# JosephCatrambone/aruco3

Measured on AMD Instinct MI355X. Metric: frames/sec at 1920x1080 ARUCO dict, higher is better.
Workload: dtype u8

## Files before the change

aruco3_amd/csrc/a3_api.hip:

```cpp
#include <algorithm>
#include <atomic>
#include <cmath>
#include <chrono>
#include <cstddef>
#include <cstdio>
#include <cstring>
#include <mutex>
#include <string>
#include <vector>

#include "a3_common.h"
#include "a3_internal.h"
#include "a3_launch.h"
#include "a3_readback.h"
#include "a3_solve_check.h"

using namespace a3;

namespace {

thread_local std::string g_create_error;

constexpr uint32_t kMaxCandDefault = 1024, kMaxCandLimit = A3_MAX_CANDIDATES_PER_FRAME;
static_assert(kMaxCandLimit == 65536, "a3_marker.candidate_index is a uint16_t");
// ... 116 lines not shown
    bool grey_valid = false;
    bool contours_valid = false;
    uint32_t tap_contours = 0; uint64_t tap_points = 0;
    bool markers_valid = false;
    uint32_t last_n = 0, last_max_per_frame = 0;
    int profiling = 0;
    int profile_every = 1;
    uint32_t batch_seq = 0;
    hipEvent_t ev[6] = {nullptr, nullptr, nullptr, nullptr, nullptr, nullptr};
    double prof_ms[A3_STAGE_COUNT] = {0, 0, 0};
    uint64_t prof_n[A3_STAGE_COUNT] = {0, 0, 0};
    a3_stats stats{};

    uint32_t W = 0, H = 0, frames = 0;

    DevBuf dict, in, grey, bin, frame_darts, frame_darts_dev, frame_base, pix_base, tile_darts;
    DevBuf d_xy, d_succ, fin, t_cur, t_next;
    DevBuf leader_list, leader_keep, entry_list, es_a, es_b;
    DevBuf contours, cyc_start_off, points;
    DevBuf cands, pre_xy, fin_xy, fin_count, work, outs, proj, patches, cand_big;
    DevBuf zero_blk;
    a3_marker* markers_ptr = nullptr;
    unsigned long long* frame_darts_ptr = nullptr;
    unsigned int* scratch_u32 = nullptr; DeviceCounters* counters = nullptr; uint32_t* per_frame = nullptr; uint32_t* frame_cursor = nullptr; uint32_t* cand_count = nullptr;
    uint32_t last_marker_total = 0;
    DevBuf tmp_a, tmp_b, tmp_c, tmp_d;
    DevBuf hsum;
    DevBuf wtab;
    DevBuf pose_buf;
    bool poses_valid = false;
    a3_refine_config refine{};
    a3_refine_config refine_prm_cfg{};
// ... 83 lines not shown
    if (bytes <= ctx->pinned_cap) return A3_OK;
    if (ctx->pinned) (void)hipHostFree(ctx->pinned);
    ctx->pinned = nullptr; ctx->pinned_cap = 0;
    A3_HIP(hipHostMalloc(&ctx->pinned, bytes, hipHostMallocDefault));
    ctx->pinned_cap = bytes;
    return A3_OK;
}

uint32_t mark_size_of(uint8_t num_bits) {
    return (uint32_t)((uint8_t)std::ceil(std::sqrt((float)num_bits)) + 2);
}

int ensure_dart_pool(a3_ctx* ctx, uint64_t darts) {
    A3_HIP(ctx->d_xy.ensure(darts * 8));
    A3_HIP(ctx->d_succ.ensure(darts * 4));
    A3_HIP(ctx->fin.ensure(darts * fin_state_bytes()));
    A3_HIP(ctx->t_cur.ensure(darts * 8));
    A3_HIP(ctx->t_next.ensure(darts * 8));
    A3_HIP(ctx->leader_list.ensure(leader_list_bytes((uint32_t)darts)));
    A3_HIP(ctx->leader_keep.ensure(leader_list_bytes((uint32_t)darts)));
    const size_t eslots = entry_slots((uint32_t)darts);
    A3_HIP(ctx->entry_list.ensure(eslots * 4));
    A3_HIP(ctx->es_a.ensure(eslots * entry_state_bytes()));
    A3_HIP(ctx->es_b.ensure(eslots * entry_state_bytes()));
    return A3_OK;
}

struct DeviceStreams { hipStream_t decode = nullptr, copy = nullptr; };
std::mutex g_streams_mu;
DeviceStreams g_dev_streams[64];
// ... 246 lines not shown
        if (b.want_pose && b.undist) A3_HIP(ctx->charuco_und.ensure(std::max<size_t>(recs, 1) * 8));
    }
    if (int rc = ensure_pinned(ctx, pinned_bytes(b.rb))) return rc;
    if (b.taps && ctx->pinned_counts_cap < (size_t)b.n * 8) {
        if (ctx->pinned_counts) (void)hipHostFree(ctx->pinned_counts);
        ctx->pinned_counts = nullptr; ctx->pinned_counts_cap = 0;
        A3_HIP(hipHostMalloc(&ctx->pinned_counts, (size_t)b.n * 8, hipHostMallocDefault));
        ctx->pinned_counts_cap = (size_t)b.n * 8;
    }
    return A3_OK;
}
int ensure_chain_buffers(a3_ctx* ctx, hipStream_t st, Batch& b, uint64_t cap_d) {
    const uint32_t n = b.n;
    const ZeroLayout z = zero_layout(1, n, n, b.marker_cap);
    A3_HIP(ctx->tile_darts.ensure(tile_darts_bytes(b.W, b.H, n)));
    A3_HIP(ctx->zero_blk.ensure(z.total));
    if (ctx->frame_darts_dev.cap < (size_t)n * 8) {
        A3_HIP(ctx->frame_darts_dev.ensure((size_t)n * 8));
        A3_HIP(hipMemsetAsync(ctx->frame_darts_dev.p, 0, ctx->frame_darts_dev.cap, st));
    }
    A3_HIP(ctx->frame_base.ensure((size_t)(n + 1) * 4));
    if (int rc = ensure_dart_pool(ctx, pool_darts_of(ctx, cap_d, 1))) return rc;
    A3_HIP(ctx->pix_base.ensure((size_t)n * b.W * b.H * 4));
    A3_HIP(ctx->contours.ensure((size_t)ctx->max_contours * sizeof(ContourRec)));
    A3_HIP(ctx->cyc_start_off.ensure((size_t)ctx->max_contours * 4));
    A3_HIP(ctx->points.ensure(ctx->max_points * 4));
    return ensure_back_buffers(ctx, b, z.head_bytes);
}


int enqueue_front(a3_ctx* ctx, Batch& b, bool held) {
    hipStream_t st = ctx->stream;
    const uint32_t n = b.n, W = b.W, H = b.H;
    const size_t npx = (size_t)W * H;
    const uint32_t kMaxCand = ctx->max_cand;
    const bool big_window = threshold_writes_grey_plane(ctx->cfg.threshold_window);
    b.need_grey = b.taps || big_window;
    b.grey_src = big_window || (b.taps && !b.sample_frames);
// ... 24 lines not shown
    if (b.prof) A3_HIP(hipEventRecord(ctx->ev[0], st));
    A3_HIP(launch_grey_threshold(st, {.pixels = b.pixels, .fmt = b.fmt, .row_stride = b.row_stride, .frame_stride = b.frame_stride, .W = (int)W, .H = (int)H,
                                      .n = n, .radius = ctx->cfg.threshold_window, .grey = b.need_grey ? ctx->grey.as<uint8_t>() : nullptr,
                                      .bits = ctx->bin.as<uint64_t>(), .hsum_tmp = big_window ? ctx->hsum.as<uint16_t>() : nullptr}));
    if (b.prof) A3_HIP(hipEventRecord(ctx->ev[1], st));
    if (!held) return A3_OK;
    A3_HIP(hipEventRecord(ctx->ev_k1_done, st));
    const uint64_t cap_d = device_plan_capacity(ctx, n, W, H);
    if (cap_d == 0) return fail(ctx, A3_ERR_INTERNAL, "a chain was held back for a batch that needs a host-side plan");
    return ensure_chain_buffers(ctx, st, b, cap_d);
}

ContourChunk contour_chunk(const a3_ctx* ctx) {
    ContourChunk c;
    c.W = (int)ctx->W; c.H = (int)ctx->H; c.batch_frames = ctx->frames;
    c.bits = ctx->bin.as<uint64_t>(); c.tile_darts = ctx->tile_darts.as<uint32_t>(); c.pix_base = ctx->pix_base.as<uint32_t>();
    c.d_rec = ctx->d_xy.as<uint64_t>(); c.d_succ = ctx->d_succ.as<uint32_t>();
    c.entry_list = ctx->entry_list.as<uint32_t>(); c.es_a = ctx->es_a.p; c.es_b = ctx->es_b.p; c.fin = ctx->fin.p;
    c.leader_count = ctx->scratch_u32 + 16; c.entry_count = ctx->scratch_u32 + 32;
    c.leader_list = ctx->leader_list.as<uint32_t>(); c.leader_keep = ctx->leader_keep.as<uint32_t>();
    c.t_cur = ctx->t_cur.as<uint64_t>(); c.t_next = ctx->t_next.as<uint64_t>();
    c.contours = ctx->contours.as<ContourRec>(); c.cyc_start_off = ctx->cyc_start_off.as<uint32_t>(); c.points = ctx->points.as<uint32_t>();
    c.max_contours = ctx->max_contours; c.max_points = ctx->max_points;
    c.cands = ctx->cands.as<CandRec>(); c.cand_count = ctx->cand_count;
    c.err_flags = ctx->scratch_u32 + 4;
    return c;
}

int enqueue_chain(a3_ctx* ctx, Batch& b, bool defer_locked) {
    hipStream_t st = ctx->stream;
    const uint32_t n = b.n, W = b.W, H = b.H;
// ... 35 lines not shown
        ctx->counters = reinterpret_cast<DeviceCounters*>(z + head_off + 256);
        ctx->per_frame = reinterpret_cast<uint32_t*>(z + head_off + 256 + ctr_bytes);
        ctx->markers_ptr = reinterpret_cast<a3_marker*>(z + head_off + head_bytes);
        zero_p = z; zero_bytes = (head_off + head_bytes + 15) & ~(size_t)15;
        return launch ? launch_zero(st, zero_p, zero_bytes) : hipSuccess;
    };
    std::vector<Chunk> chunks;
    std::vector<uint64_t> fd;
    if (device_plan) {
        if (int rc = ensure_chain_buffers(ctx, st, b, cap_d)) return rc;
        chunks.push_back(Chunk{0, n, cap_d, (uint32_t)std::min<uint64_t>(cap_d, 0xFFFFFFFFu)});
        A3_HIP(layout_zero_block(1, n, false));
        ctx->frame_darts_ptr = ctx->frame_darts_dev.as<unsigned long long>();
    } else {
        A3_HIP(ctx->tile_darts.ensure(tile_darts_bytes(W, H, n)));
        ctx->frame_darts_ptr = ctx->frame_darts.as<unsigned long long>();
        A3_HIP(hipMemsetAsync(ctx->frame_darts.p, 0, (size_t)n * 8, st));
    }
    DartCountLaunch count{.bits = ctx->bin.as<uint64_t>(), .W = (int)W, .H = (int)H, .n_frames = n, .frame_darts = ctx->frame_darts_ptr,
                          .tile_darts = ctx->tile_darts.as<uint32_t>(), .plan_cap = cap_d};
    if (device_plan) { count.frame_base = ctx->frame_base.as<uint32_t>(); count.plan = ctx->scratch_u32 + 8; count.zero_p = zero_p; count.zero_bytes = zero_bytes; }
    A3_HIP(launch_dart_count(st, count));
    const uint32_t* n_live = device_plan ? ctx->scratch_u32 + 8 : nullptr;
    uint32_t max_chunk_frames = n;
    if (!device_plan) {
        if (int rc = ensure_pinned(ctx, std::max<size_t>((size_t)n * 8, 1 << 16))) return rc;
        A3_HIP(hipMemcpyAsync(ctx->pinned, ctx->frame_darts.p, (size_t)n * 8, hipMemcpyDeviceToHost, st));
        A3_HIP(wait_stream(st));
        fd.assign((uint64_t*)ctx->pinned, (uint64_t*)ctx->pinned + n);
        uint64_t biggest = 0;
        for (uint64_t v : fd) { biggest = std::max(biggest, v); ctx->stats.darts += v; }
        if (biggest > kHardMaxDarts) return fail(ctx, A3_ERR_LIMIT, "a frame needs more contour-graph nodes than 32-bit indices allow");
        if (biggest > ctx->max_darts) ctx->max_darts = biggest;
        Chunk c{0, 0, 0, 0};
        for (uint32_t f = 0; f < n; f++) {
            if (c.count && (c.darts + fd[f] > ctx->max_darts || c.count >= kMaxChunkFrames)) { chunks.push_back(c); c = Chunk{f, 0, 0, 0}; }
            c.count++; c.darts += fd[f]; c.max_frame_darts = (uint32_t)std::max<uint64_t>(c.max_frame_darts, fd[f]);
        }
        if (c.count) chunks.push_back(c);
        max_chunk_frames = 0; uint64_t max_chunk_darts = 0;
        for (auto& c : chunks) { max_chunk_frames = std::max(max_chunk_frames, c.count); max_chunk_darts = std::max(max_chunk_darts, c.darts); }
        if (int rc = ensure_dart_pool(ctx, pool_darts_of(ctx, max_chunk_darts, chunks.size()))) return rc;
        A3_HIP(ctx->pix_base.ensure((size_t)max_chunk_frames * npx * 4));
        A3_HIP(ctx->frame_base.ensure((size_t)(max_chunk_frames + 1) * 4 * chunks.size()));
        A3_HIP(layout_zero_block(chunks.size(), max_chunk_frames, true));
        A3_HIP(ctx->contours.ensure((size_t)ctx->max_contours * sizeof(ContourRec)));
        A3_HIP(ctx->cyc_start_off.ensure((size_t)ctx->max_contours * 4));
        A3_HIP(ctx->points.ensure(ctx->max_points * 4));
        std::vector<uint32_t> bases;
        for (auto& c : chunks) {
            uint32_t acc = 0;
            for (uint32_t i = 0; i < max_chunk_frames + 1; i++) {
                bases.push_back(acc);
                if (i < c.count) acc += (uint32_t)fd[c.first + i];
            }
        }
        if (int rc = ensure_pinned(ctx, (size_t)n * 8 + bases.size() * 4 + (1 << 16))) return rc;
        uint32_t* h_bases = reinterpret_cast<uint32_t*>((uint8_t*)ctx->pinned + (size_t)n * 8);
// ... 390 lines not shown
        for (size_t i = 0; i < g_deferred.size(); i++)
            if (g_deferred[i] == ctx) { g_deferred.erase(g_deferred.begin() + (long)i); break; }
        ctx->back_deferred = false;
        for (size_t i = 0; i < g_held.size(); i++)
            if (g_held[i] == ctx) { g_held.erase(g_held.begin() + (long)i); break; }
        ctx->rest_held = false;
    }
    if (ctx->stream && ctx->stream != ctx->own_stream) (void)hipStreamSynchronize(ctx->stream);
    {
        DeviceStreams ds;
        { std::lock_guard<std::mutex> lk(g_streams_mu); ds = g_dev_streams[ctx->device & 63]; }
        if (ds.decode) (void)hipStreamSynchronize(ds.decode);
        if (ds.copy) (void)hipStreamSynchronize(ds.copy);
    }
    if (ctx->own_stream) (void)hipStreamSynchronize(ctx->own_stream);
    DevBuf* bufs[] = {&ctx->dict, &ctx->in, &ctx->grey, &ctx->bin, &ctx->frame_darts, &ctx->frame_darts_dev, &ctx->frame_base, &ctx->pix_base,
                      &ctx->tile_darts, &ctx->d_xy, &ctx->d_succ, &ctx->fin, &ctx->t_cur, &ctx->t_next,
                      &ctx->leader_list, &ctx->leader_keep, &ctx->entry_list, &ctx->es_a, &ctx->es_b,
                      &ctx->contours, &ctx->cyc_start_off, &ctx->points, &ctx->zero_blk, &ctx->cands,
                      &ctx->pre_xy, &ctx->fin_xy, &ctx->fin_count, &ctx->work, &ctx->outs, &ctx->proj, &ctx->patches, &ctx->cand_big,
                      &ctx->tmp_a, &ctx->tmp_b, &ctx->tmp_c, &ctx->tmp_d, &ctx->hsum, &ctx->pose_buf, &ctx->wtab, &ctx->refined_buf,
                      &ctx->board_slot_of, &ctx->board_slot_rec, &ctx->board_buf, &ctx->undist_buf, &ctx->charuco_tab, &ctx->charuco_tmp,
                      &ctx->charuco_buf, &ctx->charuco_und, &ctx->charuco_pose_buf, &ctx->solve_in,
                      &ctx->solve_scratch, &ctx->solve_big, &ctx->solve_out, &ctx->rect_in, &ctx->rect_out};
    for (DevBuf* b : bufs) b->release();
    if (ctx->pinned) (void)hipHostFree(ctx->pinned);
    if (ctx->pinned_counts) (void)hipHostFree(ctx->pinned_counts);
    for (auto& ev : ctx->ev) if (ev) (void)hipEventDestroy(ev);
    if (ctx->ev_in) (void)hipEventDestroy(ctx->ev_in);
    if (ctx->ev_contours) (void)hipEventDestroy(ctx->ev_contours);
    if (ctx->ev_k1) (void)hipEventDestroy(ctx->ev_k1);
    if (ctx->ev_gate) (void)hipEventDestroy(ctx->ev_gate);
// ... 325 lines not shown
    for (int r = 0; r < reps; r++) {
        A3_HIP(hipMemsetAsync(cc.leader_count, 0, 4 * 32, st));
        A3_HIP(hipEventRecord(e0, st));
        if (kernel == 0) {
            A3_HIP(hipMemsetAsync(ctx->frame_darts.p, 0, (size_t)ctx->frames * 8, st));
            A3_HIP(launch_dart_count(st, {.bits = cc.bits, .W = cc.W, .H = cc.H, .n_frames = ctx->frames, .frame_darts = ctx->frame_darts.as<unsigned long long>(),
                                          .tile_darts = ctx->tile_darts.as<uint32_t>()}));
        } else if (kernel == 1) {
            cc.dbg = dbg ? dbg : 5;
            A3_HIP(launch_dart_build(st, cc));
        } else if (kernel == 2) {
            cc.dbg = dbg ? dbg : 11;
            A3_HIP(launch_rank_cycles(st, cc));
        } else if (kernel == 3 || kernel == 4) {
            if (kernel == 4) {
                const size_t sweep = std::min<size_t>(ctx->pix_base.cap & ~(size_t)15, (size_t)512 << 20);
                if (sweep) A3_HIP(launch_zero(st, ctx->pix_base.p, sweep));
                A3_HIP(hipEventRecord(e0, st));
            }
            DecodeStage dec = decode_stage(ctx);
            dec.src = ctx->dbg_src; dec.W = cc.W; dec.H = cc.H; dec.max_cand = ctx->max_cand; dec.few = ctx->frames <= 64u; dec.grid_blocks = 4096;
            dec.per_frame = nullptr;
            dec.projection = dbg >= 0; dec.variant = dbg < 0 ? -dbg : dbg;
            A3_HIP(launch_decode(st, dec));
        } else return fail(ctx, A3_ERR_INVALID, "kernel: 0 dart_count, 1 dart_assign, 2 local_contract, 3 decode, 4 decode on cold frames");
        A3_HIP(hipEventRecord(e1, st));
        A3_HIP(hipStreamSynchronize(ctx->stream));
        float ms = 0;
        A3_HIP(hipEventElapsedTime(&ms, e0, e1));
        total += ms;
    }
    *avg_ms = (float)(total / reps);
// ... 1016 lines not shown
```

aruco3_amd/csrc/a3_launch.h:

```cpp
#pragma once

#include "a3_common.h"

namespace a3 {

struct ThresholdLaunch {
    const uint8_t* pixels = nullptr; int fmt = 0; size_t row_stride = 0, frame_stride = 0; int W = 0, H = 0; uint32_t n = 0, radius = 0;
    uint8_t* grey = nullptr; uint64_t* bits = nullptr; uint16_t* hsum_tmp = nullptr;
};
hipError_t launch_grey_threshold(hipStream_t st, const ThresholdLaunch& t);
bool threshold_writes_grey_plane(uint32_t radius);
hipError_t launch_k1_r1(hipStream_t st, const ThresholdLaunch& t);
hipError_t launch_k1_r2(hipStream_t st, const ThresholdLaunch& t);
bool ring_kernel_applies(uint32_t radius);
hipError_t launch_ring_threshold(hipStream_t st, const ThresholdLaunch& t);

size_t tile_darts_bytes(uint32_t W, uint32_t H, uint32_t n_frames);
struct DartCountLaunch {
    const uint64_t* bits = nullptr; int W = 0, H = 0; uint32_t first_frame = 0, n_frames = 0; unsigned long long* frame_darts = nullptr;
    uint32_t* tile_darts = nullptr; uint64_t plan_cap = 0; uint32_t* frame_base = nullptr; uint32_t* plan = nullptr; void* zero_p = nullptr;
    size_t zero_bytes = 0;
};
hipError_t launch_dart_count(hipStream_t st, const DartCountLaunch& d);
hipError_t launch_zero(hipStream_t st, void* p, size_t bytes);

size_t entry_state_bytes();
size_t fin_state_bytes();
size_t entry_slots(uint32_t n_darts);
size_t leader_list_bytes(uint32_t n_darts);

struct ContourChunk {
    uint32_t first_frame = 0, n_frames = 0, n_darts = 0; const uint32_t* frame_base = nullptr; DeviceCounters* ctr = nullptr;
    int max_rounds = 0;
    uint32_t* frame_entries = nullptr;
    unsigned int* dead_count = nullptr;
    int W = 0, H = 0;
    uint32_t batch_frames = 0;
    const uint64_t* bits = nullptr; const uint32_t* tile_darts = nullptr;
    const uint32_t* n_live = nullptr;
    uint32_t* pix_base = nullptr; uint64_t* d_rec = nullptr; uint32_t* d_succ = nullptr; uint32_t* entry_list = nullptr;
    unsigned int* entry_count = nullptr, * leader_count = nullptr;
    void* es_a = nullptr, * es_b = nullptr;
    void* fin = nullptr;
    uint32_t* leader_list = nullptr, * leader_keep = nullptr; uint64_t* t_cur = nullptr, * t_next = nullptr;
    int resolve_iters = 0;
    int inline_resolve_W = 0;
    uint32_t min_edge_length = 0; double eps_factor = 0.0; ContourRec* contours = nullptr; uint32_t* cyc_start_off = nullptr;
    uint32_t* points = nullptr; uint32_t max_contours = 0; uint64_t max_points = 0;
    bool keep_all = false;
    CandRec* cands = nullptr;
    uint32_t* cand_count = nullptr; uint32_t max_cand = 0; unsigned int* err_flags = nullptr;
    int phase = 0, dbg = 0;
};
hipError_t launch_dart_build(hipStream_t st, const ContourChunk& c);
hipError_t launch_rank_cycles(hipStream_t st, const ContourChunk& c);
// ... 128 lines not shown
```

aruco3_amd/csrc/k_contours.hip:

```cpp
#include <algorithm>
#include <cmath>

#include "a3_common.h"
#include "a3_launch.h"


namespace a3 {

constexpr int kFinB = 8;
constexpr int kScatB = 1;

struct Nb8 { uint64_t c; uint64_t n[8]; };

__device__ __forceinline__ uint64_t ldw(const uint64_t* __restrict__ img, int wpr, int H, int j, int y) {
    return (y >= 0 && y < H && j >= 0 && j < wpr) ? img[(size_t)y * wpr + j] : 0ull;
}

__device__ __forceinline__ void pdart_words(const Nb8& nb, uint64_t p[8]) {
#pragma unroll
    for (int k = 0; k < 8; k++) {
        uint64_t m = nb.c & nb.n[k] & ~nb.n[(k + 7) & 7];
        if ((k & 1) == 0) m &= ~nb.n[(k + 6) & 7];
        p[k] = m;
    }
// ... 11 lines not shown
    A3_DPP_ADD(0x143, 0xC)
#undef A3_DPP_ADD
    if (lane == 63) s_wave[wave] = inc;
    __syncthreads();
    uint32_t base = 0, tot = 0;
#pragma unroll
    for (int w = 0; w < 4; w++) {
        const uint32_t t = s_wave[w];
        if (w < wave) base += t;
        tot += t;
    }
    *total = tot;
    return base + inc - v;
}

constexpr int kTileWords = 4, kTileRows = 64;
__host__ __device__ inline uint32_t dart_tiles_x(uint32_t W) { return (words_per_row(W) + kTileWords - 1) / kTileWords; }
__host__ __device__ inline uint32_t dart_tiles(uint32_t W, uint32_t H) { return dart_tiles_x(W) * ((H + kTileRows - 1) / kTileRows); }

__device__ __forceinline__ void tile_stage(const uint64_t* __restrict__ img, int W, int H, uint32_t tile, uint64_t (*s_t)[kTileWords + 2]) {
    const int wpr = (int)words_per_row((uint32_t)W);
    const int tx = tile % dart_tiles_x((uint32_t)W), ty = tile / dart_tiles_x((uint32_t)W);
    const int j0 = tx * kTileWords - 1, y0 = ty * kTileRows - 1;
    constexpr int kStage = (kTileRows + 2) * (kTileWords + 2);
    static_assert(kStage <= 512, "two words per lane");
    uint64_t v[2];
#pragma unroll
    for (int k = 0; k < 2; k++) {
        const int i = min((int)threadIdx.x + 256 * k, kStage - 1);
        const int r = i / (kTileWords + 2), c = i - r * (kTileWords + 2);
        const int jj = j0 + c, yy = y0 + r;
// ... 259 lines not shown
            uint32_t first = 0;
            for (uint32_t b = 0; b < 8; b++) if (rr & (1u << b)) { first = b + 1; break; }
            kE = (5 + first - 1) & 7;
        }
        t.v[F] = (uint16_t)(P | (kW << 8) | (kE << 12));
    }
    return t;
}
__device__ __constant__ const PixLut kPixLut = make_pix_lut();

__device__ __forceinline__ int dir_dx(int k) { return (int)((0x1A90u >> (2 * k)) & 3u) - 1; }
__device__ __forceinline__ int dir_dy(int k) { return (int)((0xA901u >> (2 * k)) & 3u) - 1; }

__global__ __launch_bounds__(256) void k_dart_assign(const uint64_t* __restrict__ bits, int W, int H, uint32_t first_frame,
                                                     const uint32_t* __restrict__ frame_base, const uint32_t* __restrict__ tile_off,
                                                     uint32_t* __restrict__ pix_base, const uint32_t* __restrict__ tile_darts,
                                                     uint64_t* __restrict__ d_rec, uint32_t* __restrict__ d_succ,
                                                     const uint32_t* __restrict__ n_live, int dbg,
                                                     const unsigned long long* __restrict__ tile_mask, uint32_t tiles, uint32_t n_frames) {
    __shared__ uint32_t s_wave[4];
    __shared__ uint64_t s_t[kTileRows + 2][kTileWords + 2];
    __shared__ uint64_t s_nodes[256];
    __shared__ uint64_t s_c0[256], s_c1[256], s_c2[256];
    __shared__ uint32_t s_dbase[256];
    __shared__ uint32_t s_mark[512];
    __shared__ uint16_t s_nbk[256];
    __shared__ uint8_t s_wofrank[256], s_rank[256], s_fr[256];
    __shared__ uint32_t s_multi;
    __shared__ uint16_t s_lut[256];
    const int wpr = (int)words_per_row((uint32_t)W);
    const uint32_t n_wg = tiles * n_frames, chunk = (n_wg + 7u) >> 3, g = (blockIdx.x & 7u) * chunk + (blockIdx.x >> 3);
    if (g >= n_wg) return;
    const uint32_t f = g / tiles, tile = g - f * tiles;
    if (tile_darts[(size_t)(first_frame + f) * tiles + tile] == 0u) return;
    if (n_live && *n_live == 0u) return;
    const uint32_t dart0 = frame_base[f] + tile_off[(size_t)(first_frame + f) * tiles + tile];
    if (dbg == 1) return;
    __shared__ uint32_t s_cnt[256];
    const unsigned long long* tm = tile_mask + ((size_t)(first_frame + f) * tiles + tile) * kCountHalves;
    static_assert(kCountHalves == 4 && kTileWords == 4 && kTileRows == 64, "four 64-bit word masks per tile, four word columns of 64 rows");
    unsigned long long cm[4];
#pragma unroll
    for (int c = 0; c < 4; c++)
        cm[c] = ((tm[0] >> (16 * c)) & 0xFFFFull) | (((tm[1] >> (16 * c)) & 0xFFFFull) << 16) | (((tm[2] >> (16 * c)) & 0xFFFFull) << 32) | (((tm[3] >> (16 * c)) & 0xFFFFull) << 48);
    const unsigned long long m0 = cm[0], m1 = cm[1], m2 = cm[2], m3 = cm[3];
    tile_stage(bits + (size_t)(first_frame + f) * wpr * H, W, H, tile, s_t);
    s_cnt[threadIdx.x] = 0;
    s_mark[threadIdx.x] = 0; s_mark[256 + threadIdx.x] = 0;
    s_lut[threadIdx.x] = kPixLut.v[threadIdx.x];
    if (threadIdx.x == 0) s_multi = 0;
    __syncthreads();
    const uint32_t a0 = (uint32_t)__popcll(m0), a1 = a0 + (uint32_t)__popcll(m1), a2 = a1 + (uint32_t)__popcll(m2), n_act = a2 + (uint32_t)__popcll(m3);
    for (uint32_t k = threadIdx.x; k < n_act; k += 256) {
        const uint32_t part = (k >= a0) + (k >= a1) + (k >= a2);
        const unsigned long long mm = part == 0 ? m0 : (part == 1 ? m1 : (part == 2 ? m2 : m3));
        const uint32_t w = part * 64u + (uint32_t)select_bit(mm, k - (part == 0 ? 0u : (part == 1 ? a0 : (part == 2 ? a1 : a2))));
        const Nb8 nb = tile_nb8(s_t, (int)(w & 63u), (int)(w >> 6));
        uint64_t p[8];
        pdart_words(nb, p);
        uint64_t nodes = 0;
        uint32_t nd = 0;
#pragma unroll
        for (int q = 0; q < 8; q++) { nd += __popcll(p[q]); nodes |= p[q]; }
        const uint64_t s1 = p[0] ^ p[1] ^ p[2], k1 = (p[0] & p[1]) | (p[2] & (p[0] ^ p[1]));
        const uint64_t s2 = p[3] ^ p[4] ^ p[5], k2 = (p[3] & p[4]) | (p[5] & (p[3] ^ p[4]));
// ... 14 lines not shown
    s_dbase[threadIdx.x] = excl_d;
    {
        const uint32_t cw = s_cnt[threadIdx.x] >> 17;
        if (cw) {
            const uint32_t k = s_rank[threadIdx.x];
            s_nbk[k] = (uint16_t)excl_n;
            if (excl_n) atomicOr(&s_mark[(excl_n - 1u) >> 5], 1u << ((excl_n - 1u) & 31u));
            const uint32_t seg = (excl_n + 63u) >> 6;
            if ((seg << 6) < excl_n + cw) s_fr[seg] = (uint8_t)k;
        }
    }
    if (dbg == 2) return;
    __syncthreads();
    if (dbg == 3) return;
    const int tx = tile % dart_tiles_x((uint32_t)W), ty = tile / dart_tiles_x((uint32_t)W);
    uint32_t* pbf = pix_base + (size_t)f * W * H;
    const bool single = __builtin_amdgcn_readfirstlane((int)s_multi) == 0;
    for (uint32_t n = threadIdx.x; n < total_n; n += 256) {
        const uint32_t seg = n >> 6;
        const uint32_t marks_below = __builtin_amdgcn_mbcnt_hi(s_mark[2u * seg + 1u], __builtin_amdgcn_mbcnt_lo(s_mark[2u * seg], 0u));
        const uint32_t kr = (uint32_t)s_fr[seg] + marks_below;
        const uint32_t w = s_wofrank[kr], r = n - (uint32_t)s_nbk[kr];
        const uint64_t m = s_nodes[w];
        const int i = select_bit(m, r);
        const int jl = w >> 6, rl = w & 63;
        const int wj = tx * kTileWords + jl, wy = ty * kTileRows + rl;
        const uint32_t F = tile_F(s_t, rl, jl, i);
        const uint32_t lut = s_lut[F];
        uint32_t P = lut & 0xFFu;
        const uint64_t below = (1ull << i) - 1ull;
        const uint32_t off = single ? (uint32_t)__popcll(m & below)
                                    : (uint32_t)__popcll(s_c0[w] & below) + 2u * (uint32_t)__popcll(s_c1[w] & below) + 4u * (uint32_t)__popcll(s_c2[w] & below);
        const int x = 64 * wj + i;
        uint32_t cur = dart0 + s_dbase[w] + off;
        if ((i == 0 || i == 63 || rl == 0 || rl == kTileRows - 1) && dbg != 4) pbf[(size_t)wy * W + x] = cur;
        const int kW = x > 0 ? (int)((lut >> 8) & 15u) : 15, kE = x + 1 < W ? (int)(lut >> 12) : 15;
        const uint32_t xy = (uint32_t)x | ((uint32_t)wy << 16);
        while (P) {
            const int k = __ffs(P) - 1;
            P &= P - 1;
            const uint32_t info = (uint32_t)k | (k == kW ? kInfoW : 0u) | (k == kE ? kInfoE : 0u);
            if (dbg != 4) d_rec[cur] = dart_rec(xy, F, info, f);
            const uint32_t rr = ((F >> k) | (F << (8 - k))) & 0xFFu;
            const int ko = (k + (31 - __clz(rr))) & 7, kin = (ko + 4) & 7;
            const int lx = jl * 64 + i + dir_dx(ko), ly = rl + dir_dy(ko);
            uint32_t succ;
            if (lx >= 0 && lx < kTileWords * 64 && ly >= 0 && ly < kTileRows) {
                const int j2 = lx >> 6, i2 = lx & 63, w2 = j2 * kTileRows + ly;
                const uint32_t P2 = (uint32_t)s_lut[tile_F(s_t, ly, j2, i2)] & 0xFFu;
                succ = cur;
                if ((P2 >> kin) & 1u) {
                    const uint64_t below2 = (1ull << i2) - 1ull;
                    const uint32_t off2 = single ? (uint32_t)__popcll(s_nodes[w2] & below2)
                                                 : (uint32_t)__popcll(s_c0[w2] & below2) + 2u * (uint32_t)__popcll(s_c1[w2] & below2) +
                                                   4u * (uint32_t)__popcll(s_c2[w2] & below2);
                    succ = dart0 + s_dbase[w2] + off2 + (uint32_t)__popc(P2 & ((1u << kin) - 1u));
                }
            } else {
                succ = kNone;
            }
            if (dbg != 4 || succ == 0x12345678u) d_succ[cur] = succ;
            cur++;
        }
    }
}

__device__ __forceinline__ uint32_t pixel_F(const uint64_t* __restrict__ img, int wpr, int H, int x, int y) {
    const int j = x >> 6, i = x & 63;
    uint32_t rows[3];
#pragma unroll
    for (int dy = -1; dy <= 1; dy++) {
        const uint64_t c = ldw(img, wpr, H, j, y + dy);
        const uint64_t l = i == 0 ? ldw(img, wpr, H, j - 1, y + dy) : 0ull;
        const uint64_t r = i == 63 ? ldw(img, wpr, H, j + 1, y + dy) : 0ull;
        rows[dy + 1] = row3(l, c, r, i);
    }
    const uint32_t top = rows[0], mid = rows[1], bot = rows[2];
    return (mid & 1u) | ((top & 7u) << 1) | ((mid & 4u) << 2) | ((bot & 4u) << 3) | ((bot & 2u) << 5) | ((bot & 1u) << 7);
}

__device__ __forceinline__ uint32_t cross_tile_succ(uint32_t d, uint64_t rec, int W, int H, int wpr, uint32_t first_frame,
                                                    const uint32_t* __restrict__ pix_base, const uint64_t* __restrict__ bits) {
    const uint32_t f = rec_frame(rec);
    const uint64_t* img = bits + (size_t)(first_frame + f) * wpr * H;
    const uint32_t* pb = pix_base + (size_t)f * W * H;
    const uint32_t xy = rec_xy(rec);
    const int x = xy & 0xFFFF, y = xy >> 16;
    const uint32_t F = rec_F(rec);
    const int k = rec_info(rec) & 7;
    const uint32_t r = ((F >> k) | (F << (8 - k))) & 0xFFu;
    const int ko = (k + (31 - __clz(r))) & 7;
    const int nx = x + dir_dx(ko), ny = y + dir_dy(ko);
    const uint32_t tP = pdart_mask(pixel_F(img, wpr, H, nx, ny));
    const int kin = (ko + 4) & 7;
    return ((tP >> kin) & 1u) ? pb[(size_t)ny * W + nx] + __popc(tP & ((1u << kin) - 1u)) : d;
}

__global__ __launch_bounds__(256) void k_dart_link(int W, int H, uint32_t first_frame, const uint32_t* __restrict__ pix_base,
                                                   const uint64_t* __restrict__ bits, const uint64_t* __restrict__ d_rec,
                                                   uint32_t* __restrict__ d_succ, uint32_t n_darts, const uint32_t* __restrict__ n_live) {
    if (n_live) n_darts = min(n_darts, *n_live);
    const int wpr = (int)words_per_row((uint32_t)W);
    constexpr int B = 8;
    const uint32_t stride = gridDim.x * blockDim.x;
    const uint32_t lane = threadIdx.x & 63u;
    for (uint32_t w0 = blockIdx.x * blockDim.x + (threadIdx.x & ~63u); w0 < n_darts; w0 += B * stride) {
        uint32_t sv[B];
#pragma unroll
        for (int u = 0; u < B; u++) sv[u] = d_succ[min(w0 + lane + (uint32_t)u * stride, n_darts - 1u)];
        uint64_t m[B];
        uint32_t total = 0;
#pragma unroll
        for (int u = 0; u < B; u++) {
            m[u] = __ballot(w0 + lane + (uint32_t)u * stride < n_darts && sv[u] == kNone);
            total += (uint32_t)__popcll(m[u]);
        }
        for (uint32_t j = lane; j < total; j += 64u) {
            uint32_t acc = 0, r = 0, su = 0;
            uint64_t mm = 0;
#pragma unroll
            for (int u = 0; u < B; u++) {
                const uint32_t c = (uint32_t)__popcll(m[u]);
                if (j >= acc && j < acc + c) { mm = m[u]; r = j - acc; su = (uint32_t)u; }
                acc += c;
            }
            const uint32_t d = w0 + (uint32_t)select_bit(mm, r) + su * stride;
            d_succ[d] = cross_tile_succ(d, d_rec[d], W, H, wpr, first_frame, pix_base, bits);
        }
    }
}

constexpr int kLT = 2048;
constexpr int kLTFrame = 1024;
constexpr uint32_t kEntryShards = 16;
constexpr uint32_t kLeaderShards = 16;
__host__ __device__ inline uint32_t leader_shard_cap(uint32_t n_darts) { return n_darts / kLeaderShards + n_darts / 64u + 262144u; }
__host__ __device__ inline uint32_t entry_shard_cap(uint32_t n_darts) {
    const uint32_t tiles = (n_darts + kLT - 1) / kLT;
    return ((tiles + kEntryShards - 1) / kEntryShards) * kLT;
}
struct EntrySpace {
    uint32_t cnt[kEntryShards], span, total;
    __device__ explicit EntrySpace(const unsigned int* __restrict__ entry_count) {
// ... 958 lines not shown
    return (int)b;
}

__global__ __launch_bounds__(256) void k_zero(uint4* __restrict__ p, uint32_t n16) {
    for (uint32_t i = blockIdx.x * blockDim.x + threadIdx.x; i < n16; i += gridDim.x * blockDim.x) p[i] = make_uint4(0u, 0u, 0u, 0u);
}
hipError_t launch_zero(hipStream_t st, void* p, size_t bytes) {
    const uint32_t n16 = (uint32_t)(bytes / 16);
    hipLaunchKernelGGL(k_zero, dim3(blocks_for(n16, 256, 256)), dim3(256), 0, st, reinterpret_cast<uint4*>(p), n16);
    return hipGetLastError();
}

static size_t tile_off_offset(uint32_t W, uint32_t H, uint32_t n_frames) { return (size_t)dart_tiles(W, H) * n_frames; }
static size_t tile_mask_offset_bytes(uint32_t W, uint32_t H, uint32_t n_frames) { return ((size_t)dart_tiles(W, H) * n_frames * 4 * (1 + kCountHalves) + 7) & ~(size_t)7; }
size_t tile_darts_bytes(uint32_t W, uint32_t H, uint32_t n_frames) { return tile_mask_offset_bytes(W, H, n_frames) + (size_t)dart_tiles(W, H) * n_frames * kCountHalves * 8; }

hipError_t launch_dart_count(hipStream_t st, const DartCountLaunch& d) {
    const uint64_t* const bits = d.bits; const int W = d.W, H = d.H; const uint32_t first_frame = d.first_frame, n_frames = d.n_frames;
    unsigned long long* const frame_darts = d.frame_darts; uint32_t* const tile_darts = d.tile_darts, * const plan = d.plan;
    const uint32_t tiles_x = dart_tiles_x((uint32_t)W), tiles_y = ((uint32_t)H + kTileRows - 1) / kTileRows;
    const uint32_t wpr = words_per_row((uint32_t)W);
    uint32_t* h1 = tile_darts + (size_t)tiles_x * tiles_y * n_frames * 2;
    unsigned long long* tmask = reinterpret_cast<unsigned long long*>(reinterpret_cast<uint8_t*>(tile_darts) + tile_mask_offset_bytes((uint32_t)W, (uint32_t)H, n_frames));
    if (wpr <= 30)
        hipLaunchKernelGGL(k_dart_count<32>, dim3((tiles_y + 1) / 2, n_frames, kCountHalves), dim3(64), 0, st, bits, W, H, first_frame, frame_darts, tile_darts, h1, tmask);
    else
        hipLaunchKernelGGL(k_dart_count<64>, dim3(((wpr + kCountLanes - 1) / kCountLanes) * tiles_y, n_frames, kCountHalves), dim3(64), 0, st, bits, W, H, first_frame,
                           frame_darts, tile_darts, h1, tmask);
    hipLaunchKernelGGL(k_tile_scan, dim3(n_frames + (plan ? 1u : 0u)), dim3(256), 0, st, tile_darts, h1, tiles_x * tiles_y, first_frame,
                       tile_darts + (size_t)tiles_x * tiles_y * n_frames, n_frames, frame_darts, (unsigned long long)d.plan_cap, d.frame_base, plan,
                       reinterpret_cast<uint4*>(d.zero_p), (uint32_t)(d.zero_bytes / 16));
    return hipGetLastError();
}

hipError_t launch_dart_build(hipStream_t st, const ContourChunk& c) {
    const uint32_t tiles = dart_tiles((uint32_t)c.W, (uint32_t)c.H);
    const uint32_t* const tile_off = c.tile_darts + tile_off_offset((uint32_t)c.W, (uint32_t)c.H, c.batch_frames);
    const unsigned long long* const tile_mask = reinterpret_cast<const unsigned long long*>(
        reinterpret_cast<const uint8_t*>(c.tile_darts) + tile_mask_offset_bytes((uint32_t)c.W, (uint32_t)c.H, c.batch_frames));
    hipLaunchKernelGGL(k_dart_assign, dim3((tiles * c.n_frames + 7u) / 8u * 8u), dim3(256), 0, st, c.bits, c.W, c.H, c.first_frame, c.frame_base, tile_off,
                       c.pix_base, c.tile_darts, c.d_rec, c.d_succ, c.n_live, c.dbg, tile_mask, tiles, c.n_frames);
    if (c.dbg && c.dbg != 5) return hipGetLastError();
    hipLaunchKernelGGL(k_dart_link, dim3(blocks_for(c.n_darts, 256, 4096)), dim3(256), 0, st, c.W, c.H, c.first_frame, c.pix_base, c.bits, c.d_rec, c.d_succ,
                       c.n_darts, c.n_live);
    return hipGetLastError();
}

size_t entry_state_bytes() { return sizeof(EntryState); }
static bool finalize_inline(bool frame_entries, bool trust_natural) { return frame_entries && trust_natural; }
size_t fin_state_bytes() { return sizeof(FinState); }
size_t entry_slots(uint32_t n_darts) { return (size_t)entry_shard_cap(n_darts) * kEntryShards; }
size_t leader_list_bytes(uint32_t n_darts) { return (size_t)leader_shard_cap(n_darts) * kLeaderShards * 4; }

hipError_t launch_rank_cycles(hipStream_t st, const ContourChunk& c) {
    const uint32_t n_darts = c.n_darts, n_frames = c.n_frames, min_edge_length = c.min_edge_length; const int W = c.W, dbg = c.dbg, phase = c.phase;
    const uint64_t* const d_rec = c.d_rec; const uint32_t* const d_succ = c.d_succ, * const n_live = c.n_live, * const frame_base = c.frame_base;
    uint32_t* const entry_list = c.entry_list, * const leader_list = c.leader_list, * const frame_entries = c.frame_entries;
    unsigned int* const entry_count = c.entry_count, * const leader_count = c.leader_count, * const dead_count = c.dead_count;
    DeviceCounters* const ctr = c.ctr;
// ... 99 lines not shown
```

Measured before the change: 390,400.

## Replace full-frame pix_base with per-tile rim table and open-dart lists for linking

Swaps the full-resolution per-pixel dart-base array for a compact per-tile rim table that holds only the border pixels. Dart assign now records, per tile, which darts have no in-tile successor. The link kernel then walks only those open darts through a block scan, instead of scanning every dart's successor to find unresolved ones. This removes large scattered writes and a full pass over d_succ, at the cost of shared atomics in assign and a binary search per open dart in link.

Result: no change. 389,700, median of 2 (-0.2%).

```diff
diff --git a/aruco3_amd/csrc/a3_api.hip b/aruco3_amd/csrc/a3_api.hip
--- a/aruco3_amd/csrc/a3_api.hip
+++ b/aruco3_amd/csrc/a3_api.hip
@@ -154,8 +154,8 @@
 
     uint32_t W = 0, H = 0, frames = 0;
 
-    DevBuf dict, in, grey, bin, frame_darts, frame_darts_dev, frame_base, pix_base, tile_darts;
-    DevBuf d_xy, d_succ, fin, t_cur, t_next;
+    DevBuf dict, in, grey, bin, frame_darts, frame_darts_dev, frame_base, rim, tile_darts, tile_open, probe_sweep;
+    DevBuf d_xy, d_succ, open_list, fin, t_cur, t_next;
     DevBuf leader_list, leader_keep, entry_list, es_a, es_b;
     DevBuf contours, cyc_start_off, points;
     DevBuf cands, pre_xy, fin_xy, fin_count, work, outs, proj, patches, cand_big;
@@ -269,6 +269,7 @@
 int ensure_dart_pool(a3_ctx* ctx, uint64_t darts) {
     A3_HIP(ctx->d_xy.ensure(darts * 8));
     A3_HIP(ctx->d_succ.ensure(darts * 4));
+    A3_HIP(ctx->open_list.ensure(darts * 4));
     A3_HIP(ctx->fin.ensure(darts * fin_state_bytes()));
     A3_HIP(ctx->t_cur.ensure(darts * 8));
     A3_HIP(ctx->t_next.ensure(darts * 8));
@@ -545,6 +546,7 @@
     const uint32_t n = b.n;
     const ZeroLayout z = zero_layout(1, n, n, b.marker_cap);
     A3_HIP(ctx->tile_darts.ensure(tile_darts_bytes(b.W, b.H, n)));
+    A3_HIP(ctx->tile_open.ensure(tile_open_bytes(b.W, b.H, n)));
     A3_HIP(ctx->zero_blk.ensure(z.total));
     if (ctx->frame_darts_dev.cap < (size_t)n * 8) {
         A3_HIP(ctx->frame_darts_dev.ensure((size_t)n * 8));
@@ -552,7 +554,7 @@
     }
     A3_HIP(ctx->frame_base.ensure((size_t)(n + 1) * 4));
     if (int rc = ensure_dart_pool(ctx, pool_darts_of(ctx, cap_d, 1))) return rc;
-    A3_HIP(ctx->pix_base.ensure((size_t)n * b.W * b.H * 4));
+    A3_HIP(ctx->rim.ensure(rim_table_bytes(b.W, b.H, n)));
     A3_HIP(ctx->contours.ensure((size_t)ctx->max_contours * sizeof(ContourRec)));
     A3_HIP(ctx->cyc_start_off.ensure((size_t)ctx->max_contours * 4));
     A3_HIP(ctx->points.ensure(ctx->max_points * 4));
@@ -607,7 +609,8 @@
 ContourChunk contour_chunk(const a3_ctx* ctx) {
     ContourChunk c;
     c.W = (int)ctx->W; c.H = (int)ctx->H; c.batch_frames = ctx->frames;
-    c.bits = ctx->bin.as<uint64_t>(); c.tile_darts = ctx->tile_darts.as<uint32_t>(); c.pix_base = ctx->pix_base.as<uint32_t>();
+    c.bits = ctx->bin.as<uint64_t>(); c.tile_darts = ctx->tile_darts.as<uint32_t>(); c.tile_open = ctx->tile_open.as<uint32_t>();
+    c.rim = ctx->rim.as<uint32_t>(); c.open_list = ctx->open_list.as<uint32_t>();
     c.d_rec = ctx->d_xy.as<uint64_t>(); c.d_succ = ctx->d_succ.as<uint32_t>();
     c.entry_list = ctx->entry_list.as<uint32_t>(); c.es_a = ctx->es_a.p; c.es_b = ctx->es_b.p; c.fin = ctx->fin.p;
     c.leader_count = ctx->scratch_u32 + 16; c.entry_count = ctx->scratch_u32 + 32;
@@ -673,6 +676,7 @@
         ctx->frame_darts_ptr = ctx->frame_darts_dev.as<unsigned long long>();
     } else {
         A3_HIP(ctx->tile_darts.ensure(tile_darts_bytes(W, H, n)));
+        A3_HIP(ctx->tile_open.ensure(tile_open_bytes(W, H, n)));
         ctx->frame_darts_ptr = ctx->frame_darts.as<unsigned long long>();
         A3_HIP(hipMemsetAsync(ctx->frame_darts.p, 0, (size_t)n * 8, st));
     }
@@ -700,7 +704,7 @@
         max_chunk_frames = 0; uint64_t max_chunk_darts = 0;
         for (auto& c : chunks) { max_chunk_frames = std::max(max_chunk_frames, c.count); max_chunk_darts = std::max(max_chunk_darts, c.darts); }
         if (int rc = ensure_dart_pool(ctx, pool_darts_of(ctx, max_chunk_darts, chunks.size()))) return rc;
-        A3_HIP(ctx->pix_base.ensure((size_t)max_chunk_frames * npx * 4));
+        A3_HIP(ctx->rim.ensure(rim_table_bytes(W, H, max_chunk_frames)));
         A3_HIP(ctx->frame_base.ensure((size_t)(max_chunk_frames + 1) * 4 * chunks.size()));
         A3_HIP(layout_zero_block(chunks.size(), max_chunk_frames, true));
         A3_HIP(ctx->contours.ensure((size_t)ctx->max_contours * sizeof(ContourRec)));
@@ -1121,8 +1125,8 @@
         if (ds.copy) (void)hipStreamSynchronize(ds.copy);
     }
     if (ctx->own_stream) (void)hipStreamSynchronize(ctx->own_stream);
-    DevBuf* bufs[] = {&ctx->dict, &ctx->in, &ctx->grey, &ctx->bin, &ctx->frame_darts, &ctx->frame_darts_dev, &ctx->frame_base, &ctx->pix_base,
-                      &ctx->tile_darts, &ctx->d_xy, &ctx->d_succ, &ctx->fin, &ctx->t_cur, &ctx->t_next,
+    DevBuf* bufs[] = {&ctx->dict, &ctx->in, &ctx->grey, &ctx->bin, &ctx->frame_darts, &ctx->frame_darts_dev, &ctx->frame_base, &ctx->rim,
+                      &ctx->tile_darts, &ctx->tile_open, &ctx->probe_sweep, &ctx->d_xy, &ctx->d_succ, &ctx->open_list, &ctx->fin, &ctx->t_cur, &ctx->t_next,
                       &ctx->leader_list, &ctx->leader_keep, &ctx->entry_list, &ctx->es_a, &ctx->es_b,
                       &ctx->contours, &ctx->cyc_start_off, &ctx->points, &ctx->zero_blk, &ctx->cands,
                       &ctx->pre_xy, &ctx->fin_xy, &ctx->fin_count, &ctx->work, &ctx->outs, &ctx->proj, &ctx->patches, &ctx->cand_big,
@@ -1478,8 +1482,9 @@
             A3_HIP(launch_rank_cycles(st, cc));
         } else if (kernel == 3 || kernel == 4) {
             if (kernel == 4) {
-                const size_t sweep = std::min<size_t>(ctx->pix_base.cap & ~(size_t)15, (size_t)512 << 20);
-                if (sweep) A3_HIP(launch_zero(st, ctx->pix_base.p, sweep));
+                const size_t sweep = std::min<size_t>(((size_t)ctx->frames * ctx->W * ctx->H * 4) & ~(size_t)15, (size_t)512 << 20);
+                A3_HIP(ctx->probe_sweep.ensure(sweep));
+                if (sweep) A3_HIP(launch_zero(st, ctx->probe_sweep.p, sweep));
                 A3_HIP(hipEventRecord(e0, st));
             }
             DecodeStage dec = decode_stage(ctx);
diff --git a/aruco3_amd/csrc/a3_launch.h b/aruco3_amd/csrc/a3_launch.h
--- a/aruco3_amd/csrc/a3_launch.h
+++ b/aruco3_amd/csrc/a3_launch.h
@@ -1,6 +1,8 @@
 #pragma once
 
 #include "a3_common.h"
+#define A3_RIM_HD __host__ __device__
+#include "a3_rim.h"
 
 namespace a3 {
 
@@ -16,6 +18,8 @@
 hipError_t launch_ring_threshold(hipStream_t st, const ThresholdLaunch& t);
 
 size_t tile_darts_bytes(uint32_t W, uint32_t H, uint32_t n_frames);
+size_t tile_open_bytes(uint32_t W, uint32_t H, uint32_t n_frames);
+size_t rim_table_bytes(uint32_t W, uint32_t H, uint32_t n_frames);
 struct DartCountLaunch {
     const uint64_t* bits = nullptr; int W = 0, H = 0; uint32_t first_frame = 0, n_frames = 0; unsigned long long* frame_darts = nullptr;
     uint32_t* tile_darts = nullptr; uint64_t plan_cap = 0; uint32_t* frame_base = nullptr; uint32_t* plan = nullptr; void* zero_p = nullptr;
@@ -38,7 +42,10 @@
     uint32_t batch_frames = 0;
     const uint64_t* bits = nullptr; const uint32_t* tile_darts = nullptr;
     const uint32_t* n_live = nullptr;
-    uint32_t* pix_base = nullptr; uint64_t* d_rec = nullptr; uint32_t* d_succ = nullptr; uint32_t* entry_list = nullptr;
+    uint32_t* tile_open = nullptr;
+    uint32_t* rim = nullptr;
+    uint32_t* open_list = nullptr;
+    uint64_t* d_rec = nullptr; uint32_t* d_succ = nullptr; uint32_t* entry_list = nullptr;
     unsigned int* entry_count = nullptr, * leader_count = nullptr;
     void* es_a = nullptr, * es_b = nullptr;
     void* fin = nullptr;
diff --git a/aruco3_amd/csrc/a3_rim.h b/aruco3_amd/csrc/a3_rim.h
--- /dev/null
+++ b/aruco3_amd/csrc/a3_rim.h
@@ -0,0 +1,25 @@
+#pragma once
+#include <cstdint>
+
+#ifndef A3_RIM_HD
+#define A3_RIM_HD
+#endif
+
+namespace a3 {
+
+constexpr int kTileWords = 4, kTileRows = 64, kTileCols = kTileWords * 64;
+
+constexpr uint32_t kRimBottom = kTileCols, kRimLeft = 2 * kTileCols, kRimRight = kRimLeft + kTileRows, kRimSlots = kRimRight + kTileRows;
+static_assert(kRimSlots == 640, "256 + 256 + 64 + 64 entries per tile");
+
+A3_RIM_HD inline bool on_tile_row_rim(int ly) { return (uint32_t)(ly - 1) >= (uint32_t)(kTileRows - 2); }
+A3_RIM_HD inline bool on_tile_col_rim(int lx) { return (uint32_t)(lx - 1) >= (uint32_t)(kTileCols - 2); }
+A3_RIM_HD inline bool on_tile_rim(int lx, int ly) { return ((int)on_tile_row_rim(ly) | (int)on_tile_col_rim(lx)) != 0; }
+A3_RIM_HD inline uint32_t rim_slot(int lx, int ly) {
+    static_assert(kTileRows == 64 && kTileCols == 256, "bit 5 of the row and bit 6 of the column tell the far side from the near one");
+    const uint32_t in_row = (((uint32_t)ly & 32u) << 3) + (uint32_t)lx;
+    const uint32_t in_col = kRimLeft + ((uint32_t)lx & 64u) + (uint32_t)ly;
+    return on_tile_row_rim(ly) ? in_row : in_col;
+}
+
+}
diff --git a/aruco3_amd/csrc/k_contours.hip b/aruco3_amd/csrc/k_contours.hip
--- a/aruco3_amd/csrc/k_contours.hip
+++ b/aruco3_amd/csrc/k_contours.hip
@@ -49,7 +49,6 @@
     return base + inc - v;
 }
 
-constexpr int kTileWords = 4, kTileRows = 64;
 __host__ __device__ inline uint32_t dart_tiles_x(uint32_t W) { return (words_per_row(W) + kTileWords - 1) / kTileWords; }
 __host__ __device__ inline uint32_t dart_tiles(uint32_t W, uint32_t H) { return dart_tiles_x(W) * ((H + kTileRows - 1) / kTileRows); }
 
@@ -339,7 +338,8 @@
 
 __global__ __launch_bounds__(256) void k_dart_assign(const uint64_t* __restrict__ bits, int W, int H, uint32_t first_frame,
                                                      const uint32_t* __restrict__ frame_base, const uint32_t* __restrict__ tile_off,
-                                                     uint32_t* __restrict__ pix_base, const uint32_t* __restrict__ tile_darts,
+                                                     uint32_t* __restrict__ rim, const uint32_t* __restrict__ tile_darts,
+                                                     uint32_t* __restrict__ tile_open, uint32_t* __restrict__ open_list,
                                                      uint64_t* __restrict__ d_rec, uint32_t* __restrict__ d_succ,
                                                      const uint32_t* __restrict__ n_live, int dbg,
                                                      const unsigned long long* __restrict__ tile_mask, uint32_t tiles, uint32_t n_frames) {
@@ -352,6 +352,7 @@
     __shared__ uint16_t s_nbk[256];
     __shared__ uint8_t s_wofrank[256], s_rank[256], s_fr[256];
     __shared__ uint32_t s_multi;
+    __shared__ uint32_t s_open;
     __shared__ uint16_t s_lut[256];
     const int wpr = (int)words_per_row((uint32_t)W);
     const uint32_t n_wg = tiles * n_frames, chunk = (n_wg + 7u) >> 3, g = (blockIdx.x & 7u) * chunk + (blockIdx.x >> 3);
@@ -373,7 +374,7 @@
     s_cnt[threadIdx.x] = 0;
     s_mark[threadIdx.x] = 0; s_mark[256 + threadIdx.x] = 0;
     s_lut[threadIdx.x] = kPixLut.v[threadIdx.x];
-    if (threadIdx.x == 0) s_multi = 0;
+    if (threadIdx.x == 0) { s_multi = 0; s_open = 0; }
     __syncthreads();
     const uint32_t a0 = (uint32_t)__popcll(m0), a1 = a0 + (uint32_t)__popcll(m1), a2 = a1 + (uint32_t)__popcll(m2), n_act = a2 + (uint32_t)__popcll(m3);
     for (uint32_t k = threadIdx.x; k < n_act; k += 256) {
@@ -418,7 +419,8 @@
     __syncthreads();
     if (dbg == 3) return;
     const int tx = tile % dart_tiles_x((uint32_t)W), ty = tile / dart_tiles_x((uint32_t)W);
-    uint32_t* pbf = pix_base + (size_t)f * W * H;
+    uint32_t* const rim_t = rim + ((size_t)f * tiles + tile) * kRimSlots;
+    uint32_t* const open_t = open_list + dart0;
     const bool single = __builtin_amdgcn_readfirstlane((int)s_multi) == 0;
     for (uint32_t n = threadIdx.x; n < total_n; n += 256) {
         const uint32_t seg = n >> 6;
@@ -437,7 +439,7 @@
                                     : (uint32_t)__popcll(s_c0[w] & below) + 2u * (uint32_t)__popcll(s_c1[w] & below) + 4u * (uint32_t)__popcll(s_c2[w] & below);
         const int x = 64 * wj + i;
         uint32_t cur = dart0 + s_dbase[w] + off;
-        if ((i == 0 || i == 63 || rl == 0 || rl == kTileRows - 1) && dbg != 4) pbf[(size_t)wy * W + x] = cur;
+        if (on_tile_rim(jl * 64 + i, rl) && dbg != 4) rim_t[rim_slot(jl * 64 + i, rl)] = cur;
         const int kW = x > 0 ? (int)((lut >> 8) & 15u) : 15, kE = x + 1 < W ? (int)(lut >> 12) : 15;
         const uint32_t xy = (uint32_t)x | ((uint32_t)wy << 16);
         while (P) {
@@ -464,9 +466,15 @@
                 succ = kNone;
             }
             if (dbg != 4 || succ == 0x12345678u) d_succ[cur] = succ;
+            if (succ == kNone) {
+                const uint32_t slot = atomicAdd(&s_open, 1u);
+                if (dbg != 4) open_t[slot] = cur;
+            }
             cur++;
         }
     }
+    __syncthreads();
+    if (threadIdx.x == 0 && dbg != 4) tile_open[(size_t)(first_frame + f) * tiles + tile] = s_open;
 }
 
 __device__ __forceinline__ uint32_t pixel_F(const uint64_t* __restrict__ img, int wpr, int H, int x, int y) {
@@ -483,11 +491,10 @@
     return (mid & 1u) | ((top & 7u) << 1) | ((mid & 4u) << 2) | ((bot & 4u) << 3) | ((bot & 2u) << 5) | ((bot & 1u) << 7);
 }
 
-__device__ __forceinline__ uint32_t cross_tile_succ(uint32_t d, uint64_t rec, int W, int H, int wpr, uint32_t first_frame,
-                                                    const uint32_t* __restrict__ pix_base, const uint64_t* __restrict__ bits) {
+__device__ __forceinline__ uint32_t cross_tile_succ(uint32_t d, uint64_t rec, int H, int wpr, uint32_t first_frame, uint32_t tiles_x, uint32_t tiles,
+                                                    const uint32_t* __restrict__ rim, const uint64_t* __restrict__ bits) {
     const uint32_t f = rec_frame(rec);
     const uint64_t* img = bits + (size_t)(first_frame + f) * wpr * H;
-    const uint32_t* pb = pix_base + (size_t)f * W * H;
     const uint32_t xy = rec_xy(rec);
     const int x = xy & 0xFFFF, y = xy >> 16;
     const uint32_t F = rec_F(rec);
@@ -497,40 +504,52 @@
     const int nx = x + dir_dx(ko), ny = y + dir_dy(ko);
     const uint32_t tP = pdart_mask(pixel_F(img, wpr, H, nx, ny));
     const int kin = (ko + 4) & 7;
-    return ((tP >> kin) & 1u) ? pb[(size_t)ny * W + nx] + __popc(tP & ((1u << kin) - 1u)) : d;
-}
-
-__global__ __launch_bounds__(256) void k_dart_link(int W, int H, uint32_t first_frame, const uint32_t* __restrict__ pix_base,
+    if (!((tP >> kin) & 1u)) return d;
+    const uint32_t ttile = (uint32_t)(ny / kTileRows) * tiles_x + (uint32_t)(nx / kTileCols);
+    return rim[((size_t)f * tiles + ttile) * kRimSlots + rim_slot(nx % kTileCols, ny % kTileRows)] + __popc(tP & ((1u << kin) - 1u));
+}
+
+constexpr uint32_t kLinkTilesPerWg = 16, kLinkMaxWgs = 2048;
+
+__global__ __launch_bounds__(256) void k_dart_link(int W, int H, uint32_t first_frame, const uint32_t* __restrict__ rim,
                                                    const uint64_t* __restrict__ bits, const uint64_t* __restrict__ d_rec,
-                                                   uint32_t* __restrict__ d_succ, uint32_t n_darts, const uint32_t* __restrict__ n_live) {
-    if (n_live) n_darts = min(n_darts, *n_live);
+                                                   uint32_t* __restrict__ d_succ, const uint32_t* __restrict__ n_live,
+                                                   const uint32_t* __restrict__ frame_base, const uint32_t* __restrict__ tile_off,
+                                                   const uint32_t* __restrict__ tile_darts, const uint32_t* __restrict__ tile_open,
+                                                   const uint32_t* __restrict__ open_list, uint32_t tiles, uint32_t n_frames) {
+    __shared__ uint32_t s_wave[4];
+    __shared__ uint32_t s_excl[256], s_first[256];
+    if (n_live && *n_live == 0u) return;
     const int wpr = (int)words_per_row((uint32_t)W);
-    constexpr int B = 8;
-    const uint32_t stride = gridDim.x * blockDim.x;
-    const uint32_t lane = threadIdx.x & 63u;
-    for (uint32_t w0 = blockIdx.x * blockDim.x + (threadIdx.x & ~63u); w0 < n_darts; w0 += B * stride) {
-        uint32_t sv[B];
-#pragma unroll
-        for (int u = 0; u < B; u++) sv[u] = d_succ[min(w0 + lane + (uint32_t)u * stride, n_darts - 1u)];
-        uint64_t m[B];
-        uint32_t total = 0;
-#pragma unroll
-        for (int u = 0; u < B; u++) {
-            m[u] = __ballot(w0 + lane + (uint32_t)u * stride < n_darts && sv[u] == kNone);
-            total += (uint32_t)__popcll(m[u]);
-        }
-        for (uint32_t j = lane; j < total; j += 64u) {
-            uint32_t acc = 0, r = 0, su = 0;
-            uint64_t mm = 0;
-#pragma unroll
-            for (int u = 0; u < B; u++) {
-                const uint32_t c = (uint32_t)__popcll(m[u]);
-                if (j >= acc && j < acc + c) { mm = m[u]; r = j - acc; su = (uint32_t)u; }
-                acc += c;
+    const uint32_t tiles_x = dart_tiles_x((uint32_t)W);
+    const uint32_t n_wg = tiles * n_frames, chunk = (n_wg + 7u) >> 3, xcd = blockIdx.x & 7u, per_xcd = gridDim.x >> 3;
+    const uint32_t per = (chunk + per_xcd - 1u) / per_xcd;
+    const uint32_t x_end = min((xcd + 1u) * chunk, n_wg);
+    const uint32_t g_begin = xcd * chunk + (blockIdx.x >> 3) * per, g_end = min(g_begin + per, x_end);
+    for (uint32_t g0 = g_begin; g0 < g_end; g0 += 256u) {
+        const uint32_t g = g0 + threadIdx.x;
+        uint32_t n_open = 0, first = 0;
+        if (g < g_end) {
+            const uint32_t f = g / tiles;
+            const size_t t = (size_t)first_frame * tiles + g;
+            if (tile_darts[t] != 0u) {
+                n_open = tile_open[t];
+                first = frame_base[f] + tile_off[t];
             }
-            const uint32_t d = w0 + (uint32_t)select_bit(mm, r) + su * stride;
-            d_succ[d] = cross_tile_succ(d, d_rec[d], W, H, wpr, first_frame, pix_base, bits);
-        }
+        }
+        uint32_t total;
+        const uint32_t excl = block_excl_scan_256(n_open, s_wave, &total);
+        s_excl[threadIdx.x] = excl; s_first[threadIdx.x] = first;
+        __syncthreads();
+        for (uint32_t j = threadIdx.x; j < total; j += 256u) {
+            uint32_t t = 0;
+#pragma unroll
+            for (uint32_t step = 128u; step; step >>= 1)
+                if (s_excl[t + step] <= j) t += step;
+            const uint32_t d = open_list[s_first[t] + (j - s_excl[t])];
+            d_succ[d] = cross_tile_succ(d, d_rec[d], H, wpr, first_frame, tiles_x, tiles, rim, bits);
+        }
+        __syncthreads();
     }
 }
 
@@ -1519,6 +1538,8 @@
 static size_t tile_off_offset(uint32_t W, uint32_t H, uint32_t n_frames) { return (size_t)dart_tiles(W, H) * n_frames; }
 static size_t tile_mask_offset_bytes(uint32_t W, uint32_t H, uint32_t n_frames) { return ((size_t)dart_tiles(W, H) * n_frames * 4 * (1 + kCountHalves) + 7) & ~(size_t)7; }
 size_t tile_darts_bytes(uint32_t W, uint32_t H, uint32_t n_frames) { return tile_mask_offset_bytes(W, H, n_frames) + (size_t)dart_tiles(W, H) * n_frames * kCountHalves * 8; }
+size_t tile_open_bytes(uint32_t W, uint32_t H, uint32_t n_frames) { return (size_t)dart_tiles(W, H) * n_frames * 4; }
+size_t rim_table_bytes(uint32_t W, uint32_t H, uint32_t n_frames) { return (size_t)dart_tiles(W, H) * n_frames * kRimSlots * 4; }
 
 hipError_t launch_dart_count(hipStream_t st, const DartCountLaunch& d) {
     const uint64_t* const bits = d.bits; const int W = d.W, H = d.H; const uint32_t first_frame = d.first_frame, n_frames = d.n_frames;
@@ -1544,10 +1565,11 @@
     const unsigned long long* const tile_mask = reinterpret_cast<const unsigned long long*>(
         reinterpret_cast<const uint8_t*>(c.tile_darts) + tile_mask_offset_bytes((uint32_t)c.W, (uint32_t)c.H, c.batch_frames));
     hipLaunchKernelGGL(k_dart_assign, dim3((tiles * c.n_frames + 7u) / 8u * 8u), dim3(256), 0, st, c.bits, c.W, c.H, c.first_frame, c.frame_base, tile_off,
-                       c.pix_base, c.tile_darts, c.d_rec, c.d_succ, c.n_live, c.dbg, tile_mask, tiles, c.n_frames);
+                       c.rim, c.tile_darts, c.tile_open, c.open_list, c.d_rec, c.d_succ, c.n_live, c.dbg, tile_mask, tiles, c.n_frames);
     if (c.dbg && c.dbg != 5) return hipGetLastError();
-    hipLaunchKernelGGL(k_dart_link, dim3(blocks_for(c.n_darts, 256, 4096)), dim3(256), 0, st, c.W, c.H, c.first_frame, c.pix_base, c.bits, c.d_rec, c.d_succ,
-                       c.n_darts, c.n_live);
+    const uint32_t link_wgs = std::min(kLinkMaxWgs, ((tiles * c.n_frames + kLinkTilesPerWg - 1u) / kLinkTilesPerWg + 7u) & ~7u);
+    hipLaunchKernelGGL(k_dart_link, dim3(link_wgs), dim3(256), 0, st, c.W, c.H, c.first_frame, c.rim, c.bits, c.d_rec, c.d_succ, c.n_live, c.frame_base,
+                       tile_off, c.tile_darts, c.tile_open, c.open_list, tiles, c.n_frames);
     return hipGetLastError();
 }
 
```
